# wejoncy/QLLM

Hardware: AMD Instinct MI355X
Metric: decode_tokens_per_s_llama2_7b_w4a16_g128_linear_stack (higher is better)
Workload: dtype f16; 1 GPU; llama2-7b-awq-w4-g128-decode-b1; pack_mode=GEMM, bits=4, group_size=128, layers=32, linears_per_layer=7, batch=1, driven_through=q_layer modules (sibling groups installed by the loader), grouped_qkv_gateup=True, weight_layout=native strip-major copy built on device at first use (qllm_repack_native), graph=True, parallelism=replicas x1, ranks_seen=1, device=gfx950, compute_units=256

## Files before the change

qllm_amd/csrc/capi.hip:

```cpp
#include <stdarg.h>
#include <stdio.h>
#include <string.h>

#include <algorithm>

#include "planner.hpp"

namespace qllm {

static thread_local char g_err[512] = {0};

int set_error(int code, const char *fmt, ...) {
  va_list ap;
  va_start(ap, fmt);
  vsnprintf(g_err, sizeof(g_err), fmt, ap);
  va_end(ap);
  return code;
}
void clear_error() { g_err[0] = 0; }
const char *last_error_text() { return g_err; }

static int native_shape_ok(int bits, int K, int N, int group_size, bool packed_zeros) {
  if (bits != 4 && bits != 3) return set_error(QLLM_ERR_UNSUPPORTED, "the native layout holds 3- and 4-bit weights (got %d)", bits);
  if (K % 32 != 0 || N % 16 != 0) return set_error(QLLM_ERR_UNSUPPORTED, "the native layout needs K %% 32 == 0 and N %% 16 == 0 (K=%d N=%d)", K, N);
// ... 21 lines not shown
    if (w->g_idx) return set_error(QLLM_ERR_INVALID, "the native layout has no act-order (g_idx must be NULL: sort the rows by group first)");
    if (w->layout == QLLM_LAYOUT_NATIVE_F16Z && !w->qzeros) return set_error(QLLM_ERR_INVALID, "NATIVE_F16Z layout needs fp16 qzeros");
  } else {
    if ((w->K * w->bits) % 32 != 0) return set_error(QLLM_ERR_INVALID, "in_features*bits must be a multiple of 32 (K=%d bits=%d)", w->K, w->bits);
    if (w->layout == QLLM_LAYOUT_HQQ && !w->qzeros) return set_error(QLLM_ERR_INVALID, "HQQ layout needs fp16 qzeros");
    if (w->layout == QLLM_LAYOUT_HQQ && w->g_idx) return set_error(QLLM_ERR_INVALID, "HQQ layout has no act-order (g_idx must be NULL)");
    if (w->layout == QLLM_LAYOUT_GPTQ && w->qzeros && (w->N * w->bits) % 32 != 0)
      return set_error(QLLM_ERR_INVALID, "out_features*bits must be a multiple of 32 for packed zeros (N=%d bits=%d)", w->N, w->bits);
  }
  if (w->add_zero_bias < 0 || w->add_zero_bias > 1) return set_error(QLLM_ERR_INVALID, "add_zero_bias must be 0 or 1");
  return QLLM_OK;
}

static int check_io(const void *x, const void *y, int M, int act_dtype) {
  if (!x || !y) return set_error(QLLM_ERR_INVALID, "x / y must not be NULL");
  if (M <= 0) return set_error(QLLM_ERR_INVALID, "M must be >= 1 (got %d)", M);
  if (act_dtype != QLLM_F16 && act_dtype != QLLM_BF16) return set_error(QLLM_ERR_INVALID, "act_dtype must be f16 or bf16");
  if ((uintptr_t)x % 16 != 0) return set_error(QLLM_ERR_INVALID, "x must be 16-byte aligned");
  return QLLM_OK;
}

static int check_quant_layer(const char *required, bool missing, int32_t w_dtype, int32_t N, int32_t K, int32_t group_size) {
  if (missing) return set_error(QLLM_ERR_INVALID, "%s must not be NULL", required);
  if (w_dtype != QLLM_F16 && w_dtype != QLLM_BF16 && w_dtype != QLLM_F32) return set_error(QLLM_ERR_INVALID, "w_dtype must be QLLM_F16, QLLM_BF16 or QLLM_F32");
  if (N <= 0 || K <= 0 || group_size <= 0) return set_error(QLLM_ERR_INVALID, "bad N/K/group_size (%d/%d/%d)", N, K, group_size);
  return QLLM_OK;
}
static int check_whole_groups(int32_t K, int32_t group_size) {
  if (K % group_size != 0) return set_error(QLLM_ERR_INVALID, "K must be a multiple of group_size (K=%d group_size=%d)", K, group_size);
  return QLLM_OK;
}
static int elem_size(int32_t w_dtype) { return w_dtype == QLLM_F32 ? 4 : 2; }
static const char *const kElemAligned = "every buffer must be aligned to its element size";

static int check_workspace(const char *entry, const void *workspace, size_t workspace_bytes, size_t need) {
  if ((need && !workspace) || workspace_bytes < need || (uintptr_t)workspace % 16)
    return set_error(QLLM_ERR_WORKSPACE, "%s needs a 16-byte aligned workspace of %zu bytes (got %zu)", entry, need, workspace ? workspace_bytes : (size_t)0);
  return QLLM_OK;
}

static uint64_t *g_timeline = nullptr;
static int g_timeline_slots = 0, g_timeline_next = 0;

static size_t usable_ws(const void *workspace, size_t workspace_bytes) {
  return (workspace && (uintptr_t)workspace % 256 == 0) ? workspace_bytes : 0;
}
static void carve(void *workspace, int **counters, float **slabs) {
  *counters = (int *)workspace;
  *slabs = (float *)((char *)workspace + kCounterBytes);
}
static void set_split(GemmParams &p, int S, void *workspace, int tail_from = 0, int tail_split = 0) {
  p.split_k = S;
  p.tail_from = tail_split > 1 ? tail_from : 0;
  p.tail_split = tail_split > 1 ? tail_split : 0;
  p.counters = nullptr;
  p.slabs = nullptr;
  if (S > 1 || tail_split > 1) carve(workspace, &p.counters, &p.slabs);
}
static void fill_launch_params(GemmParams &p, const qllm_weight_t *w, const void *x, void *y, int M, int act_dtype) {
  fill_gemm_params(p, w, x, y, M, act_dtype);
#ifdef QLLM_LAB
  p.dbg = g_timeline;
#endif
}

static int fill_strip1_params(Strip1Params &p, const qllm_weight_t *w, void *const *y, int n, const void *x, int M, int act_dtype) {
  fill_call(p, w[0], x, M, act_dtype);
  p.T = w[0].K / 32;
  p.n_groups = w[0].K / w[0].group_size;
  p.group64 = w[0].group_size == 64;
  p.bits3 = w[0].bits == 3;
  int max_strips = 0;
  for (int i = 0; i < n; ++i) {
    fill_layer(p.prob[i], w[i], y[i]);
    p.prob[i].n_strips = w[i].N / 16;
    max_strips = std::max(max_strips, p.prob[i].n_strips);
  }
  return max_strips;
}
static int run_strip1(const StripPlan &pl, const qllm_weight_t *w, void *const *y, int n, const void *x, int M, int act_dtype, hipStream_t stream) {
  Strip1Params p;
  const int max_strips = fill_strip1_params(p, w, y, n, x, M, act_dtype);
  p.dbg = (g_timeline && g_timeline_next < g_timeline_slots) ? g_timeline + 24 * (g_timeline_next++) : nullptr;
  return launch_strip1(p, pl.one_nw, pl.one_maxs, n, max_strips, stream);
}

static int run_strip(const StripPlan &pl, const qllm_weight_t *w, void *const *y, int n, const void *x, int M, int act_dtype, hipStream_t stream) {
  if (pl.one_nw) return run_strip1(pl, w, y, n, x, M, act_dtype, stream);
  StripParams p;
  fill_call(p, w[0], x, M, act_dtype);
  p.n_prob = n;
  p.K = w[0].K;
  p.T = w[0].K / 32;
  p.cpl = pl.cpl;
  p.bits = w[0].bits;
  p.nw = pl.nw;
  p.spw = pl.spw;
  p.ra = pl.ra;
  p.sm = pl.sm;
  p.n_groups = (w[0].K + w[0].group_size - 1) / w[0].group_size;
  p.group_size = w[0].group_size;
  p.dbg = (pl.sm && (!pl.ra || pl.ra == 2) && p.bits == 4 && p.group_size == 128 && g_timeline && g_timeline_next < g_timeline_slots)
              ? g_timeline + 24 * (g_timeline_next++) : nullptr;
  int block = 0;
  for (int i = 0; i < n; ++i) {
    StripProblem &q = p.prob[i];
    fill_layer(q, w[i], y[i]);
    q.N = w[i].N;
    q.n_strips = (w[i].N / 16 + pl.cpl - 1) / pl.cpl;
    q.block_begin = block;
    p.block_begin8[i] = block;
    block += q.n_strips;
  }
  return launch_strip(p, block, stream);
}

static int run_skinny(const qllm_weight_t *w, void *const *y, int n, const void *x, int M, int act_dtype, void *workspace,
                      size_t workspace_bytes, hipStream_t stream) {
  const SkinnyPlan s = plan_skinny(w, n, M);
  if (s.tiles_total > (int)(kCounterBytes / sizeof(int))) return set_error(QLLM_ERR_UNSUPPORTED, "too many column tiles (%d)", s.tiles_total);

  SkinnyParams p;
  fill_call(p, w[0], x, M, act_dtype);
  p.n_prob = n;
  p.K = w[0].K;
  p.T = w[0].K / 32;
  p.group_size = w[0].group_size;
  size_t slab_off = kCounterBytes;
  int tile_off = 0, block = 0;
  for (int i = 0; i < n; ++i) {
    SkinnyProblem &q = p.prob[i];
    fill_layer(q, w[i], y[i]);
    q.N = w[i].N;
    q.n_tiles = (w[i].N + s.tile_cols - 1) / s.tile_cols;
    q.S = s.S;
    q.spw = s.spw;
    q.block_begin = block;
    q.counters = (int *)workspace + tile_off;
    q.slabs = (float *)((char *)workspace + slab_off);
    tile_off += q.n_tiles;
    block += q.n_tiles * s.S;
    if (s.S > 1) slab_off += align_up((size_t)s.S * M * w[i].N * sizeof(float), 256);
  }
  if (s.S > 1) {
    if (!workspace) return set_error(QLLM_ERR_WORKSPACE, "split-K needs a workspace (call qllm_workspace_bytes)");
    if (workspace_bytes < slab_off) return set_error(QLLM_ERR_WORKSPACE, "workspace too small: need %zu bytes, have %zu", slab_off, workspace_bytes);
    if ((uintptr_t)workspace % 256 != 0) return set_error(QLLM_ERR_INVALID, "workspace must be 256-byte aligned");
  }
  return launch_skinny(p, w[0].layout, s.awq_w, block, stream);
}

static const char kNotPrefillKernel[] = "QLLM_F16_IN_BF16_OUT: M=%d K=%d N=%d is not served by the 256x128 prefill kernel";
static int run_tile_gemm(GemmParams &p, int layout, void *workspace, size_t workspace_bytes, hipStream_t stream, bool bf16_out_only = false) {
  const TileChoice c = choose_tile(p, layout, usable_ws(workspace, workspace_bytes));
  if (bf16_out_only && c.kernel != 3) return set_error(QLLM_ERR_UNSUPPORTED, kNotPrefillKernel, p.M, p.K, p.N);
  set_split(p, c.split_k, workspace, c.tail_from, c.tail_split);
  if (c.kernel == 2 && p.N % 128 != 0)
    return set_error(QLLM_ERR_WORKSPACE, "N %% 128 == 64 with bf16 activations converted to fp16: the workspace must hold the copy (call qllm_workspace_bytes_act)");
  if (c.kernel == 2) return launch_gemm2(p, layout, stream);
  if (bf16_out_only) p.out_bf16 = 1;
  if (c.native_bf16) {
    p.native_bf16 = 1;
    p.act_bf16 = 0;
  } else if (p.act_bf16) {
    void *xh = (char *)workspace + c.copy_off;
    if (int rc = launch_bf16_to_f16(p.x, xh, (size_t)p.M * p.K, stream)) return rc;
// ... 459 lines not shown
```

qllm_amd/csrc/kernels.hpp:

```cpp
#pragma once
#include "common.hpp"

namespace qllm {

int launch_dequant(const qllm_weight_t &w, int zero_kind, void *out, int out_dtype, int out_transposed, hipStream_t stream);
int launch_unpack_qweight(const void *qweight, int layout, int bits, int K, int N, int32_t *q_kn, hipStream_t stream);
int launch_pack_qweight(const int32_t *q_kn, int layout, int bits, int K, int N, void *qweight, hipStream_t stream);

int launch_ort_dequant(const void *qweight, const void *scales, const void *qzeros, int zeros_f16, const int32_t *g_idx,
                       int block, int K, int N, void *out, hipStream_t stream);

constexpr int kMaxProblems = 8;

struct SkinnyProblem {
  const uint32_t *qweight;
  const half_t *scales;
  const void *qzeros;
  const half_t *bias;
  void *y;
  float *slabs;
  int *counters;
  int N;
  int n_tiles;
  int S;
// ... 46 lines not shown
  int n_groups;
  int sm;
  uint64_t *dbg;
};
bool strip_group_ok(int group_size, bool strip_major, int bits);
int strip_nw(int K, int strips_total, int compute_units);
int strip_sm_nw(int K, int M, int group_size, int bits);
int strip_spw(int K, int group_size, int nw);
int strip_maxs(int nw, int spw, int cpl, int ra, int sm);
int strip_xl(int nw, int M, int spw, int cpl, int sm);
size_t strip_lds_bytes(int M, int spw, int nw, int cpl, int group_size, int ra, int sm);
int strip_cpl(int cols_total, bool all_mult64, bool all_mult32, int compute_units);
bool strip_x_ok(int M, int spw, int nw, int cpl, int sm);
int launch_strip(const StripParams &p, int grid, hipStream_t stream);
int launch_strip_sm(const StripParams &p, int grid, hipStream_t stream);
int launch_strip_sm_ra(const StripParams &p, int grid, hipStream_t stream);
int launch_strip_dma_g32(const StripParams &p, int grid, hipStream_t stream);
int launch_strip_dma_g64(const StripParams &p, int grid, hipStream_t stream);
int launch_strip_dma_g128(const StripParams &p, int grid, hipStream_t stream);

struct Strip1Problem {
  const uint32_t *qweight;
  const half_t *scales;
  const void *qzeros;
  const half_t *bias;
  void *y;
  int n_strips;
  int zero_kind;
};
struct Strip1Params {
  const void *x;
  int T;
  int n_groups;
  int group64;
  int M;
  int bits3;
  int add_zero_bias;
  int act_bf16;
  uint64_t *dbg;
  Strip1Problem prob[kMaxProblems];
  void *const *ar_peers;
  int *ar_status;
  int ar_rank, ar_world;
  uint32_t ar_slot_bytes;
};

constexpr int kBitGemvMaxM = 16;
struct BitGemvParams {
  const void *x;
  const uint32_t *qweight;
  const half_t *scales;
  const void *qzeros;
  const half_t *bias;
  void *y;
  float *slabs;
  int *counters;
  int M, K, N, group_size, zero_kind, add_zero_bias, act_bf16;
  int ksplit;
  int n_col_blocks, chunk_units;
};
bool bitgemv_ok(const qllm_weight_t &w, int M);
int bitgemv_split(int M, int K, int N);
int bitgemv_cols();
int launch_bitgemv(const BitGemvParams &p, int bits, hipStream_t stream);

constexpr int kCommMaxWorld = 16;
struct CommCtl {
  uint32_t flag[2][kCommMaxWorld];
  uint32_t epoch;
  uint32_t ticket;
};
__device__ __forceinline__ void store16_sys(void *p, uint4_t v) {
  __hip_atomic_store((uint64_t *)p, ((uint64_t)v.y << 32) | v.x, __ATOMIC_RELAXED, __HIP_MEMORY_SCOPE_SYSTEM);
  __hip_atomic_store((uint64_t *)p + 1, ((uint64_t)v.w << 32) | v.z, __ATOMIC_RELAXED, __HIP_MEMORY_SCOPE_SYSTEM);
}
__device__ __forceinline__ uint4_t load16_sys(const void *p) {
  const uint64_t a = __hip_atomic_load((const uint64_t *)p, __ATOMIC_RELAXED, __HIP_MEMORY_SCOPE_SYSTEM);
  const uint64_t b = __hip_atomic_load((const uint64_t *)p + 1, __ATOMIC_RELAXED, __HIP_MEMORY_SCOPE_SYSTEM);
  return uint4_t{(uint32_t)a, (uint32_t)(a >> 32), (uint32_t)b, (uint32_t)(b >> 32)};
}
bool strip1_shape(int K, int blocks, int cus, int *nw, int *maxs, bool odd64 = false);
int launch_strip1(const Strip1Params &p, int nw, int maxs, int n_prob, int max_strips, hipStream_t stream);
int launch_strip1_allreduce(const Strip1Params &p, int nw, int maxs, int n_strips, hipStream_t stream);

int launch_repack_native(const qllm_weight_t &src, int zero_kind, void *qweight_out, void *scales_out, void *qzeros_out, hipStream_t stream);
int launch_unpack_native(const qllm_weight_t &src, int dst_layout, void *qweight_out, void *scales_out, void *qzeros_out, hipStream_t stream);

bool gather_columns_ok(int K);
int launch_gather_columns(const void *x, const int32_t *perm, void *out, int M, int K, hipStream_t stream);

struct GemmParams {
  const void *x;
  const uint32_t *qweight;
  const half_t *scales;
  const void *qzeros;
  const int32_t *g_idx;
  const half_t *bias;
  void *y;
  int M, K, N, group_size, gs_shift, add_zero_bias, zero_kind, act_bf16, n_groups;
  int raster;
  int stagger;
  int out_bf16;
  int sm;
  int split_k;
  float *slabs;
  int *counters;
  int tail_from, tail_split;
  int n_prob, total_tiles;
  struct GemmProb {
    const uint32_t *qweight;
    const half_t *scales;
    const void *qzeros;
    const half_t *bias;
    void *y;
    int N, zero_kind, tile_begin, pad_;
  } prob[4];
  int native_bf16;
  int prio;
  uint64_t *dbg;
};
int launch_gemm(const GemmParams &p, int layout, hipStream_t stream);

bool gemm2_ok(const GemmParams &p, int layout);
int gemm2_split_k(int M, int N, int K);
constexpr int kGemm3MaxProb = 4;
using GemmProb = GemmParams::GemmProb;
int gemm3_tail_split(int M, int N, int K, int *tail_from);
int gemm3_tail_split_tiles(int tiles, int K, int *tail_from, bool uneven = false);
bool gemm3_bf16_native(int layout);
int gemm2_tile_n(int M, int N, int split_k);
size_t gemm2_slab_bytes(int M, int N, int S);
int launch_gemm2(const GemmParams &p, int layout, hipStream_t stream);

struct PanelProblem {
  const uint32_t *qweight;
  const half_t *scales;
  const void *qzeros;
  const half_t *bias;
  void *y;
  int N, zero_kind, panel_begin, pad_;
};
struct PanelParams {
  const void *x;
  int M, K, n_groups, group_size, bits, add_zero_bias, act_bf16, n_prob, split_k, abl, n_panels;
  float *slabs;
  int *counters;
  PanelProblem prob[kMaxProblems];
};
bool panel_shape_ok(int M, int K, int N, int group_size, int bits);
int panel_mt(int M);
int panel_kh(int M);
int panel_split_k(int M, int n_panels, int K);
size_t panel_slab_bytes(int M, int n_panels, int S);
int launch_panel(const PanelParams &p, hipStream_t stream);

constexpr int kGemm3Rows3Bit = 100;
bool gemm3_ok(const GemmParams &p, int layout);
bool gemm3_n_tail(const GemmParams &p, int layout);
inline int gemm3_tile_cols(int N) { return (N + 127) / 128 * 128; }
int gemm3_split_k(int M, int N, int K);
int launch_gemm3(const GemmParams &p, int layout, hipStream_t stream);
int launch_bf16_to_f16(const void *src, void *dst, size_t n, hipStream_t stream);

bool hqq_quant_shape_ok(int N, int K, int bits, int group_size);
size_t hqq_quant_workspace_bytes(int N, int K, int group_size, int iters);
int launch_hqq_quantize(const void *w_nk, int w_dtype, int N, int K, int bits, int group_size, int iters, float lp_norm, float beta, float kappa,
// ... 23 lines not shown
```

qllm_amd/csrc/planner.hip:

```cpp
#include <stdio.h>
#include <stdlib.h>
#include <string.h>

#include <algorithm>

#include "planner.hpp"

namespace qllm {

static int env_int(const char *name, int dflt) {
  const char *v = getenv(name);
  return (v && *v) ? atoi(v) : dflt;
}
static Settable kSettable[] = {
    {"QLLM_STRIP1_3BIT", 0, 1, 0, 0},
    {"QLLM_STRIP1_MAX_M", 1, 4, 0, 0},
    {"QLLM_STRIP1", 0, 2, 0, 0},
    {"QLLM_PANEL", 0, 1, 0, 0},
    {"QLLM_PANEL_MIN_M", 17, 129, 0, 0},
    {"QLLM_PANEL_GROUP_MIN_M", 17, 129, 0, 0},
    {"QLLM_GEMM2", 0, 1, 0, 0},
    {"QLLM_GEMM3", 0, 1, 0, 0},
    {"QLLM_GEMM2_MIN_M", 33, 1 << 30, 0, 0},
    {"QLLM_GEMM3_MIN_M", 0, 1 << 30, 0, 0},
    {"QLLM_GEMM2_SPLITK", 0, 1, 0, 0},
    {"QLLM_GEMM3_TAIL", 0, 1, 0, 0},
    {"QLLM_GEMM3_GROUP", 0, 1, 0, 0},
    {"QLLM_GEMM3_BF16", 0, 1, 0, 0},
    {"QLLM_SKINNY_MAX_M", 0, 64, 0, 0},
    {"QLLM_STRIP_MIN", 0, 1 << 20, 0, 0},
    {"QLLM_BITGEMV", 0, 1, 0, 0},
};
int g_knob_overrides = 0;
Settable *find_knob(const char *name) {
  for (Settable &k : kSettable)
    if (strcmp(k.name, name) == 0) return &k;
  return nullptr;
}
void reset_knobs() {
  for (Settable &k : kSettable) k.set = 0;
  __atomic_store_n(&g_knob_overrides, 0, __ATOMIC_RELAXED);
}
int knob_override(const char *name, int dflt) {
  for (const Settable &k : kSettable)
    if (k.set && strcmp(k.name, name) == 0) return k.value;
  return dflt;
}
#ifdef QLLM_LAB
int knob(const char *name, int dflt) { return g_knob_overrides ? knob_override(name, env_int(name, dflt)) : env_int(name, dflt); }
#endif
int compute_units() {
  static int v = [] {
    int e = env_int("QLLM_NUM_CU", 0);
    if (e > 0) return e;
    int dev = 0, n = 0;
    if (hipGetDevice(&dev) == hipSuccess && hipDeviceGetAttribute(&n, hipDeviceAttributeMultiprocessorCount, dev) == hipSuccess && n > 0) return n;
    (void)hipGetLastError();
    return kNumCU;
  }();
  return v;
}
static int skinny_target_waves() { return knob("QLLM_SKINNY_WAVES", 2048); }
static int skinny_awq_w(int M) { return (M <= 16 && knob("QLLM_SKINNY_AWQ_W", 1) == 2) ? 2 : 1; }
static int skinny_max_m() { return std::min(knob("QLLM_SKINNY_MAX_M", 64), 64); }
static int strip_min_strips() {
  return knob("QLLM_STRIP_MIN", 8);
}

static bool ptrs_aligned(const qllm_weight_t &w) {
  return (uintptr_t)w.qweight % 16 == 0 && (uintptr_t)w.scales % 16 == 0 && (!w.qzeros || (uintptr_t)w.qzeros % 8 == 0);
}
static bool fused_common_ok(const qllm_weight_t &w) {
  return !is_native(w) && w.bits == 4 && w.N % 8 == 0 && w.group_size % 8 == 0 && ptrs_aligned(w);
}
static bool skinny_ok(const qllm_weight_t &w, int M) {
  return M <= skinny_max_m() && fused_common_ok(w) && w.K % 32 == 0 && w.g_idx == nullptr;
}
static bool gemm_ok(const qllm_weight_t &w) {
  if (!fused_common_ok(w) || w.K % 64 != 0) return false;
  if (w.layout == QLLM_LAYOUT_AWQ_GEMM) return w.group_size % 4 == 0;
  if (w.g_idx) {
    const int groups = (w.K + w.group_size - 1) / w.group_size;
    return (size_t)groups * 128 * 4 + 65536 <= 160 * 1024;
  }
  return true;
}
static int layout_family(const qllm_weight_t &w) { return is_native(w) ? 2 : (w.layout == QLLM_LAYOUT_AWQ_GEMM ? 1 : 0); }

void fill_gemm_params(GemmParams &p, const qllm_weight_t *w, const void *x, void *y, int M, int act_dtype) {
  fill_call(p, *w, x, M, act_dtype);
  fill_layer(p, *w, y);
  p.g_idx = w->g_idx;
  p.K = w->K;
  p.N = w->N;
  p.group_size = w->group_size;
  p.gs_shift = ((w->group_size & (w->group_size - 1)) == 0) ? __builtin_ctz((unsigned)w->group_size) : -1;
  p.n_groups = (w->K + w->group_size - 1) / w->group_size;
  p.sm = is_native(*w) ? 1 : 0;
  p.split_k = 1;
// ... 116 lines not shown
  for (int ci = 0; ci < n_cands; ++ci) {
    const int c = cands[ci];
    if (!dma_fits(c)) continue;
    int blocks = 0;
    for (int i = 0; i < n; ++i) blocks += (w[i].N / 16 + c - 1) / c;
    const double cost = (double)((blocks + cus - 1) / cus) * (96.0 * 1024 + x_bytes + c * strip_bytes);
    if (best == 0 || cost < best_cost * 0.97) { best = c; best_cost = cost; }
    if (c == dma_cpl) { best = c; break; }
  }
  const int cpl = best ? best : 1;
  const bool g32_ra = g32 && cpl == 1 && M <= 8 && K <= 4096;
  const int nw = (cpl == 1 && M <= 16) ? 16 : 8;
  const int spw = (strip_spw(K, gs, nw) + 1) & ~1;
  if (g32_ra || strip_lds_bytes(M, spw, nw, cpl, gs, 2, 1) > 156 * 1024) return false;
  return take(plan, cpl, nw, spw, 2, 1);
}

static void upgrade_to_strip1(const qllm_weight_t &w, int M, int strips, StripPlan *plan) {
  int nw1 = 0, maxs1 = 0;
  const int s1 = knob("QLLM_STRIP1", 1);
  const bool w4 = w.bits == 4 && (w.group_size == 128 || (w.group_size == 64 && s1 != 2 && w.K <= 24576));
  const bool w3 = w.bits == 3 && (w.group_size == 128 || w.group_size == 64) && w.K <= 16384 && knob("QLLM_STRIP1_3BIT", 1);
  if (M == 1 && (w4 || w3) && s1 && strip1_shape(w.K, strips, compute_units(), &nw1, &maxs1, w4 && w.group_size == 64)) {
    plan->one_nw = nw1;
    plan->one_maxs = maxs1;
  }
}
static bool plan_strip_native(const qllm_weight_t *w, int M, const StripCols &c, bool after_dma, StripPlan *plan) {
  const int K = w[0].K, gs = w[0].group_size, bits = w[0].bits;
  const bool g32 = gs == 32;
  const bool longk = strip_longk(w[0]);
  const int slab_nw = strip_ra_base(M) ? 0 : strip_sm_nw(K, M, gs, bits);
  const int sm_ra_cpl4 = knob("QLLM_SM_RA_CPL4", 1);
  const int cpl = (!after_dma && sm_ra_cpl4 && !g32 && slab_nw == 0 && M >= 5 && M <= 16 && c.m64 && c.cols / 64 >= compute_units() / 2) ? (bits == 3 ? 2 : 4) : 1;
  int nw = after_dma ? (M > 16 ? 8 : 16) : ((M > 16 || cpl > 1) ? 8 : (slab_nw ? slab_nw : 16));
  for (int tries = 0; tries < 2; ++tries) {
    const int spw = strip_spw(K, gs, nw);
    const int ra = (slab_nw == 0 || (longk && nw == 16)) ? 1 : 0;
    if (!ra && K / 32 < strip_maxs(nw, spw, 1, 0, 1)) return false;
    if ((ra || strip_x_ok(M, spw, nw, 1, 1)) && strip_lds_bytes(M, spw, nw, cpl, gs, ra, 1) <= 156 * 1024) {
      upgrade_to_strip1(w[0], M, c.cols / 16, plan);
      return take(plan, cpl, nw, spw, ra, 1);
    }
    if (nw == 16 || M > 16 || cpl > 1) break;
    nw = 16;
  }
  return false;
}

static bool plan_strip_rowstream(const qllm_weight_t *w, int M, const StripCols &c, StripPlan *plan) {
  const int K = w[0].K, gs = w[0].group_size, bits = w[0].bits, cus = compute_units();
  const int ra_base = strip_ra_base(M);
  const bool longk = strip_longk(w[0]);
  int force_cpl = knob("QLLM_STRIP_CPL", 0);
  int first = (bits == 3 || M > 16) ? 1 : strip_cpl(c.cols, c.m64, c.m32 && M <= 4, cus);
  if (M > 16) force_cpl = 1;
  if (force_cpl == 4 && c.m64 && bits == 4) first = 4;
  if (force_cpl == 2 && c.m32 && bits == 4) first = 2;
  if (force_cpl == 1) first = 1;
  const int cand_cpl[2] = {first, 1};
  for (int ci = 0; ci < 2; ++ci) {
    const int cpl = cand_cpl[ci];
    if (ci >= 1 && cpl == cand_cpl[ci - 1]) continue;
    const int strips = c.cols / (16 * cpl);
    if (cpl == 1 && strips < strip_min_strips()) continue;
    int nw = cpl == 4 ? 8 : ((cpl == 2 || bits == 3) ? 16 : strip_nw(K, strips, cus));
    if (M > 16) nw = 8;
    for (int tries = 0; tries < 2; ++tries) {
      const int spw = strip_spw(K, gs, nw);
      const int ra = (ra_base || (longk && cpl == 1 && nw == 16)) ? 1 : 0;
      if ((ra || strip_x_ok(M, spw, nw, cpl, 0)) && strip_lds_bytes(M, spw, nw, cpl, gs, ra, 0) <= 156 * 1024) return take(plan, cpl, nw, spw, ra, 0);
      if (nw == 16 || M > 16 || cpl == 4) break;
      nw = 16;
    }
  }
  return false;
}

bool strip_plan(const qllm_weight_t *w, int n, int M, StripPlan *plan) {
  *plan = StripPlan{};
  StripCols c;
  if (M > strip_row_limit(w, n) || panel_takes_instead(w, n, M) || !strip_layers_ok(w, n, M, &c)) return false;
  if (!is_native(w[0])) return plan_strip_rowstream(w, M, c, plan);
  if (plan_strip1_rows4(w, M, c.cols / 16, plan)) return true;
  const bool dma = strip_dma_applies(w, n, M);
  if (dma && plan_strip_dma(w, n, M, plan)) return true;
  return plan_strip_native(w, M, c, dma, plan);
}

SkinnyPlan plan_skinny(const qllm_weight_t *w, int n, int M) {
  SkinnyPlan s;
  s.awq_w = skinny_awq_w(M);
  s.tile_cols = skinny_tile_cols(w[0].layout, s.awq_w);
  s.tiles_total = 0;
  for (int i = 0; i < n; ++i) s.tiles_total += (w[i].N + s.tile_cols - 1) / s.tile_cols;
  skinny_plan(w[0].K, M, s.tiles_total, skinny_target_waves(), &s.S, &s.spw);
  return s;
}

static bool split_fits(size_t ws_bytes, size_t slab_bytes, int counters) {
  return ws_bytes >= kCounterBytes + slab_bytes && counters <= (int)(kCounterBytes / sizeof(int));
}
int gemm3_split_for(int M, int N, int K, size_t ws_bytes) {
  const int S = gemm3_split_k(M, N, K);
  if (S <= 1 || !split_fits(ws_bytes, gemm2_slab_bytes(M, gemm3_tile_cols(N), S), tiles_256x128(M, gemm3_tile_cols(N)))) return 1;
  return S;
}
static int gemm2_split_for(int M, int N, int K, size_t ws_bytes) {
  const int S = gemm2_split_k(M, N, K);
  if (S <= 1 || !split_fits(ws_bytes, gemm2_slab_bytes(M, N, S), tiles_256x128(M, N))) return 1;
  return S;
}
int panel_split_for(int M, int n_panels, int K, size_t ws_bytes) {
  const int S = panel_split_k(M, n_panels, K);
  if (S <= 1 || !split_fits(ws_bytes, panel_slab_bytes(M, n_panels, S), n_panels)) return 1;
  return S;
}
int bitgemv_split_for(int M, int K, int N, size_t ws_bytes) {
  const int S = bitgemv_split(M, K, N);
  if (S <= 1 || !split_fits(ws_bytes, (size_t)S * M * N * sizeof(float), (N + 15) / 16)) return 1;
  return S;
}
static size_t gemm3_tail_slab_bytes(int tail_tiles, int TS) { return TS > 1 ? (size_t)tail_tiles * TS * 256 * 128 * sizeof(float) : 0; }
static int tail_that_fits(int TS, int tiles, size_t ws_bytes, int *tail_from) {
  if (TS > 1 && split_fits(ws_bytes, gemm3_tail_slab_bytes(tiles - *tail_from, TS), tiles - *tail_from)) return TS;
  *tail_from = tiles;
  return 1;
}
static int gemm3_tail_for(int M, int N, int K, size_t ws_bytes, int *tail_from) {
  return tail_that_fits(gemm3_tail_split(M, N, K, tail_from), tiles_256x128(M, gemm3_tile_cols(N)), ws_bytes, tail_from);
}
static int group_tiles(const qllm_weight_t *w, int n, int M) {
  int t = 0;
  for (int i = 0; i < n; ++i) t += tiles_256x128(M, w[i].N);
  return t;
}
int tile_group_tail_for(const qllm_weight_t *w, int n, int M, size_t ws_bytes, int *tail_from) {
  const int tiles = group_tiles(w, n, M);
  return tail_that_fits(gemm3_tail_split_tiles(tiles, w[0].K, tail_from), tiles, ws_bytes, tail_from);
}

static size_t bf16_copy_bytes(int M, int K, int act_bf16) { return act_bf16 ? align_up((size_t)M * K * 2, 256) : 0; }

TileChoice choose_tile(const GemmParams &p, int layout, size_t ws_bytes) {
  GemmParams q = p;
  q.act_bf16 = 0;
  if (gemm3_ok(q, layout)) {
    const int S3 = gemm3_split_for(p.M, p.N, p.K, ws_bytes);
    if (gemm2_split_k(p.M, p.N, p.K) == 1 || S3 > 1) {
      const int native = p.act_bf16 && gemm3_bf16_native(layout);
      const size_t copy = native ? 0 : bf16_copy_bytes(p.M, p.K, p.act_bf16);
      const int tiles = tiles_256x128(p.M, gemm3_tile_cols(p.N));
      int tail_from = tiles;
      const int TS = S3 > 1 ? 1 : gemm3_tail_for(p.M, p.N, p.K, ws_bytes > copy ? ws_bytes - copy : 0, &tail_from);
      const size_t used = kCounterBytes + (S3 > 1 ? align_up(gemm2_slab_bytes(p.M, gemm3_tile_cols(p.N), S3), 256) : align_up(gemm3_tail_slab_bytes(tiles - tail_from, TS), 256));
      if (!copy || ws_bytes >= used + copy) return TileChoice{3, S3, used, tail_from, TS, native};
    }
  }
  return TileChoice{2, gemm2_split_for(p.M, p.N, p.K, ws_bytes), 0, 0, 0, 0};
}

static bool native_prefill_ok(const qllm_weight_t *w, GemmParams &p) {
  if (!ptrs_aligned(*w)) return false;
  if (panel_serves(w, p.M)) return true;
  if (w->bits == 3) return gemm3_ok(p, kGemm3Rows3Bit);
  if (w->bits != 4) return false;
  if (gemm2_ok(p, QLLM_LAYOUT_GPTQ)) return true;
  GemmParams q = p;
  q.act_bf16 = 0;
  return gemm3_n_tail(q, QLLM_LAYOUT_GPTQ) && gemm3_ok(q, QLLM_LAYOUT_GPTQ);
}

static Decision routed(Route r, int layout = 0) {
  Decision d;
  memset(&d, 0, sizeof(d));
  d.route = r;
  d.layout = layout;
  return d;
}
static Decision refused(int rc) {
  Decision d = routed(ROUTE_NONE);
  d.rc = rc;
  return d;
}

Decision decide_single(const qllm_weight_t *w, int M, int act_dtype) {
  Decision d = routed(ROUTE_STRIP);
  GemmParams p;
  fill_gemm_params(p, w, nullptr, nullptr, M, act_dtype);
  if ((w->bits == 3 || is_native(*w)) && strip_plan(w, 1, M, &d.strip)) return d;
  if (is_native(*w)) {
    if (!native_prefill_ok(w, p))
      return refused(set_error(QLLM_ERR_UNSUPPORTED, "native-layout layer: no fused kernel for M=%d K=%d N=%d g=%d bits=%d (decode sizes, and M > 64 with "
                               "K %% 64 == 0, N %% 128 == 0 and a power-of-two group size, are served)", M, w->K, w->N, w->group_size, w->bits));
    if (panel_serves(w, M)) return routed(ROUTE_PANEL);
    if (w->bits == 3) return routed(ROUTE_ROWS3, kGemm3Rows3Bit);
    return routed(ROUTE_TILE, QLLM_LAYOUT_GPTQ);
  }
  if (skinny_ok(*w, M)) {
    if (strip_plan(w, 1, M, &d.strip)) return d;
    if (M > 32 && gemm_ok(*w) && gemm2_ok(p, w->layout)) return routed(ROUTE_TILE, w->layout);
    return routed(ROUTE_SKINNY);
  }
  if (w->bits == 3 && M > 64 && w->layout != QLLM_LAYOUT_AWQ_GEMM && !w->g_idx && ptrs_aligned(*w) && gemm3_ok(p, kGemm3Rows3Bit))
    return routed(ROUTE_ROWS3, kGemm3Rows3Bit);
  if (gemm_ok(*w)) return routed(gemm2_ok(p, w->layout) ? ROUTE_TILE : ROUTE_GEMM, w->layout);
  if (knob("QLLM_BITGEMV", 1) && bitgemv_ok(*w, M)) return routed(ROUTE_BITGEMV);
  return refused(set_error(QLLM_ERR_UNSUPPORTED, "no fused kernel for bits=%d K=%d N=%d g=%d layout=%d act_order=%d; use qllm_dequant + GEMM",
                           w->bits, w->K, w->N, w->group_size, w->layout, w->g_idx != nullptr));
}

static bool tile_group_serves(const qllm_weight_t *w, int n, int M, int act_dtype) {
  if (!knob("QLLM_GEMM3_GROUP", 1) || !knob("QLLM_GEMM3", 1) || n < 2 || n > kGemm3MaxProb || M < 384) return false;
  const int gs = w[0].group_size;
  if (w[0].bits != 4 || w[0].K % 64 != 0 || gs < 32 || (gs & (gs - 1)) != 0) return false;
  if (act_dtype == QLLM_BF16 && !gemm3_bf16_native(QLLM_LAYOUT_GPTQ)) return false;
  for (int i = 0; i < n; ++i) {
    if (w[i].layout == QLLM_LAYOUT_AWQ_GEMM || w[i].g_idx || w[i].N % 128 != 0 || is_native(w[i]) != is_native(w[0])) return false;
    if (!ptrs_aligned(w[i])) return false;
    if ((size_t)M * w[i].K * 2 >= 0x7fffffffull || (size_t)w[i].K * w[i].N / 2 >= 0x7fffffffull) return false;
  }
  return group_tiles(w, n, M) >= compute_units();
}

Decision decide_group(const qllm_weight_t *w, int n, int M, int act_dtype) {
  for (int i = 0; i < n; ++i) {
    if (w[i].K != w[0].K || w[i].group_size != w[0].group_size || w[i].bits != w[0].bits || layout_family(w[0]) != layout_family(w[i]) ||
        w[i].add_zero_bias != w[0].add_zero_bias)
      return refused(set_error(QLLM_ERR_INVALID, "grouped weights must agree on K, group_size, bits, layout family and add_zero_bias"));
  }
  if (tile_group_serves(w, n, M, act_dtype)) return routed(ROUTE_TILE_GROUP, QLLM_LAYOUT_GPTQ);
  for (int i = 0; i < n; ++i) {
    if (w[i].bits == 3 || is_native(w[i])) continue;
    if (!skinny_ok(w[i], M))
      return refused(set_error(QLLM_ERR_UNSUPPORTED, "grouped forward needs the decode kernel (4-bit, M<=%d, K%%32==0, no act-order)", skinny_max_m()));
  }
  Decision d = routed(ROUTE_STRIP);
  if (strip_plan(w, n, M, &d.strip)) return d;
  if (panel_group_serves(w, n, M)) return routed(ROUTE_PANEL);
  if (is_native(w[0]))
    return refused(set_error(QLLM_ERR_UNSUPPORTED, "grouped forward: native-layout layers are served for M <= 32 (4 bits: <= 128) with group size 64 / 128 (4 bits: also 32), and 4-bit groups of at least one 256x128 tile per CU from 384 rows (M=%d g=%d)", M, w[0].group_size));
  if (w[0].bits != 4) return refused(set_error(QLLM_ERR_UNSUPPORTED, "grouped forward: no fused kernel for %d-bit weights in this shape", w[0].bits));
  return routed(ROUTE_SKINNY);
}

void describe(const Decision &d, const qllm_weight_t *w, int n, int M, size_t ws_bytes, char *buf, size_t buflen) {
  const char *sm = is_native(w[0]) ? " layout=strip-major" : "";
  switch (d.route) {
    case ROUTE_STRIP: {
      const StripPlan &pl = d.strip;
      if (pl.one_nw)
        snprintf(buf, buflen, "strip1 nw=%d round=%d%s%s%s grid=strips x %d layout=strip-major", pl.one_nw, pl.one_maxs,
                 pl.one_nw * pl.one_maxs == w[0].K / 32 ? " exact" : "", w[0].group_size == 64 ? (w[0].bits == 3 ? " g64 bits=3" : " g64") : (w[0].bits == 3 ? " bits=3" : ""),
                 M > 1 ? " rows=4" : "", n);
      else
        snprintf(buf, buflen, "strip nw=%d cpl=%d spw=%d form=%s row_tiles=%d%s", pl.nw, pl.cpl, pl.spw,
                 pl.ra == 2 ? "dma-A" : (pl.ra ? "register-A" : "lds-slab"), M > 32 ? 4 : (M > 16 ? 2 : 1), pl.sm ? " layout=strip-major" : "");
      return;
    }
    case ROUTE_PANEL: {
      char layers[24] = "";
      if (n > 1) snprintf(layers, sizeof(layers), " layers=%d", n);
      snprintf(buf, buflen, "panel cols=64 row_tiles=%d k_halves=%d split_k=%d%s%s layout=strip-major", panel_mt(M), panel_kh(M),
               panel_split_for(M, panels_of(w, n), w[0].K, ws_bytes), layers, w[0].bits == 3 ? " bits=3" : "");
      return;
    }
    case ROUTE_ROWS3: {
      const int S = gemm3_split_for(M, w[0].N, w[0].K, ws_bytes);
      if (S > 1) snprintf(buf, buflen, "gemm3 tile=256x128 matrix-waves=8 staging-waves=4 bits=3 split_k=%d%s", S, sm);
      else snprintf(buf, buflen, "gemm3 tile=256x128 matrix-waves=8 staging-waves=4 bits=3%s", sm);
      return;
    }
    case ROUTE_TILE: {
      GemmParams p;
      fill_gemm_params(p, &w[0], nullptr, nullptr, M, QLLM_F16);
      const TileChoice c = choose_tile(p, d.layout, ws_bytes);
      const char *nt = w[0].N % 128 ? " n_tail=64" : "";
      if (c.kernel == 3 && c.tail_split > 1) snprintf(buf, buflen, "gemm3 tile=256x128 matrix-waves=8 staging-waves=4 tail_split=%d%s%s", c.tail_split, nt, sm);
      else if (c.kernel == 3 && c.split_k > 1) snprintf(buf, buflen, "gemm3 tile=256x128 matrix-waves=8 staging-waves=4 split_k=%d%s%s", c.split_k, nt, sm);
      else if (c.kernel == 3) snprintf(buf, buflen, "gemm3 tile=256x128 matrix-waves=8 staging-waves=4%s%s", nt, sm);
      else snprintf(buf, buflen, "gemm2 tile=256x%d split_k=%d%s", gemm2_tile_n(M, w[0].N, c.split_k), c.split_k, sm);
      return;
    }
    case ROUTE_TILE_GROUP: {
      int tail_from = 0;
      const int TS = tile_group_tail_for(w, n, M, ws_bytes, &tail_from);
      if (TS > 1) snprintf(buf, buflen, "gemm3 tile=256x128 matrix-waves=8 staging-waves=4 layers=%d tail_split=%d%s", n, TS, sm);
      else snprintf(buf, buflen, "gemm3 tile=256x128 matrix-waves=8 staging-waves=4 layers=%d%s", n, sm);
      return;
    }
    case ROUTE_GEMM: snprintf(buf, buflen, "gemm tile=128x128%s", w[0].g_idx ? " act-order-gather" : ""); return;
    case ROUTE_SKINNY: {
      const SkinnyPlan s = plan_skinny(w, n, M);
      snprintf(buf, buflen, "skinny tile_cols=%d split_k=%d spw=%d", s.tile_cols, s.S, s.spw);
      return;
    }
    case ROUTE_BITGEMV:
      snprintf(buf, buflen, "bitgemv bits=%d cols=%d waves=8 split_k=%d", w[0].bits, bitgemv_cols(), bitgemv_split_for(M, w[0].K, w[0].N, ws_bytes));
      return;
    default: snprintf(buf, buflen, "unsupported (%s)", last_error_text()[0] ? last_error_text() : "dequant + GEMM");
  }
}

size_t workspace_bytes_act(const qllm_weight_t *w, int M, int act_dtype) {
  if (!w || M <= 0) return kCounterBytes;
  size_t tiles = 0;
  if (M > 32) {
    GemmParams p;
    fill_gemm_params(p, w, nullptr, nullptr, M, QLLM_F16);
    p.g_idx = nullptr;
    const bool g3 = gemm3_ok(p, w->bits == 3 ? kGemm3Rows3Bit : (w->layout == QLLM_LAYOUT_AWQ_GEMM ? QLLM_LAYOUT_AWQ_GEMM : QLLM_LAYOUT_GPTQ));
    int tail_from = 0;
    const int TS = g3 && w->bits != 3 ? gemm3_tail_split(M, w->N, w->K, &tail_from) : 1;
    const size_t tail = align_up(gemm3_tail_slab_bytes(tiles_256x128(M, gemm3_tile_cols(w->N)) - tail_from, TS), 256);
    const size_t split3 = g3 ? align_up(gemm2_slab_bytes(M, gemm3_tile_cols(w->N), gemm3_split_k(M, w->N, w->K)), 256) : 0;
    tiles = std::max(std::max(align_up(gemm2_slab_bytes(M, w->N, gemm2_split_k(M, w->N, w->K)), 256), split3), tail) +
            (g3 ? bf16_copy_bytes(M, w->K, act_dtype == QLLM_BF16) : 0);
    if (M > 128) return kCounterBytes + tiles;
  }
  if (M >= 9 && M <= 128 && w->N % 64 == 0) tiles = std::max(tiles, align_up(panel_slab_bytes(M, w->N / 64, panel_split_k(M, w->N / 64, w->K)), 256));
  if (M > 64) return kCounterBytes + tiles;
  const size_t slabs = align_up((size_t)skinny_max_split(M) * M * w->N * sizeof(float), 256);
  return kCounterBytes + (tiles > slabs ? tiles : slabs);
}

}
```

qllm_amd/csrc/planner.hpp:

```cpp
#pragma once
#include <string.h>

#include "kernels.hpp"

namespace qllm {

constexpr size_t kCounterBytes = 16384;
inline size_t align_up(size_t v, size_t a) { return (v + a - 1) / a * a; }
const char *last_error_text();

struct Settable {
  const char *name;
  int lo, hi;
  int value, set;
};
Settable *find_knob(const char *name);
void reset_knobs();
inline int panel_ablation() { return knob("QLLM_PANEL_ABL", 0); }

inline bool is_native(const qllm_weight_t &w) { return w.layout == QLLM_LAYOUT_NATIVE || w.layout == QLLM_LAYOUT_NATIVE_F16Z; }
inline int zero_kind_of(const qllm_weight_t &w) {
  if (w.layout == QLLM_LAYOUT_HQQ || w.layout == QLLM_LAYOUT_NATIVE_F16Z) return ZK_F16;
  if (w.qzeros == nullptr) return ZK_SYM;
  return ZK_PACKED;
}
template <typename Params>
inline void fill_call(Params &p, const qllm_weight_t &w0, const void *x, int M, int act_dtype) {
  memset(&p, 0, sizeof(p));
  p.x = x;
  p.M = M;
  p.add_zero_bias = w0.add_zero_bias;
  p.act_bf16 = (act_dtype == QLLM_BF16);
}
template <typename Problem>
inline void fill_layer(Problem &q, const qllm_weight_t &w, void *y) {
  q.qweight = (const uint32_t *)w.qweight;
  q.scales = (const half_t *)w.scales;
  q.qzeros = w.qzeros;
  q.bias = (const half_t *)w.bias;
  q.y = y;
  q.zero_kind = zero_kind_of(w);
}
inline int tiles_256x128(int M, int cols) { return ((M + 255) / 256) * (cols / 128); }
void fill_gemm_params(GemmParams &p, const qllm_weight_t *w, const void *x, void *y, int M, int act_dtype);

struct StripPlan {
  int cpl, nw, spw, ra, sm;
  int one_nw, one_maxs;
};
bool strip_plan(const qllm_weight_t *w, int n, int M, StripPlan *plan);

struct SkinnyPlan {
  int awq_w, tile_cols, tiles_total, S, spw;
};
SkinnyPlan plan_skinny(const qllm_weight_t *w, int n, int M);

struct TileChoice {
  int kernel;
  int split_k;
  size_t copy_off;
  int tail_from, tail_split;
  int native_bf16;
};
TileChoice choose_tile(const GemmParams &p, int layout, size_t ws_bytes);

int gemm3_split_for(int M, int N, int K, size_t ws_bytes);
int panel_split_for(int M, int n_panels, int K, size_t ws_bytes);
int bitgemv_split_for(int M, int K, int N, size_t ws_bytes);
int tile_group_tail_for(const qllm_weight_t *w, int n, int M, size_t ws_bytes, int *tail_from);

enum Route { ROUTE_NONE = 0, ROUTE_STRIP, ROUTE_PANEL, ROUTE_ROWS3, ROUTE_TILE, ROUTE_GEMM, ROUTE_SKINNY, ROUTE_BITGEMV, ROUTE_TILE_GROUP };
struct Decision {
  Route route;
  StripPlan strip;
  int layout;
  int rc;
};
Decision decide_single(const qllm_weight_t *w, int M, int act_dtype);
Decision decide_group(const qllm_weight_t *w, int n, int M, int act_dtype);
void describe(const Decision &d, const qllm_weight_t *w, int n, int M, size_t ws_bytes, char *buf, size_t buflen);
size_t workspace_bytes_act(const qllm_weight_t *w, int M, int act_dtype);

}
```

Baseline: 1155 tokens/s.

## Add strip1 walk kernel issuing all grouped members' weight loads at once

Adds a specialised strip1 kernel for grouped launches of two or three 4-bit g128 members (QKV, gate/up). Each block loads every member's weights, scales and zeros into registers up front, then reuses one prepared activation slab in LDS across all members. The goal is more memory-level parallelism and less repeated activation preparation in decode GEMV. The cost is higher register and LDS pressure, plus extra template instantiations. The planner enables it by default through a knob.

```diff
diff --git a/qllm_amd/csrc/capi.hip b/qllm_amd/csrc/capi.hip
--- a/qllm_amd/csrc/capi.hip
+++ b/qllm_amd/csrc/capi.hip
@@ -127,6 +127,7 @@
   Strip1Params p;
   const int max_strips = fill_strip1_params(p, w, y, n, x, M, act_dtype);
   p.dbg = (g_timeline && g_timeline_next < g_timeline_slots) ? g_timeline + 24 * (g_timeline_next++) : nullptr;
+  if (pl.one_walk > 0 && !p.dbg) return launch_strip1_walk(p, pl.one_nw, pl.one_maxs, n, max_strips, stream);
   return launch_strip1(p, pl.one_nw, pl.one_maxs, n, max_strips, stream);
 }
 
diff --git a/qllm_amd/csrc/kernels.hpp b/qllm_amd/csrc/kernels.hpp
--- a/qllm_amd/csrc/kernels.hpp
+++ b/qllm_amd/csrc/kernels.hpp
@@ -152,6 +152,8 @@
 bool strip1_shape(int K, int blocks, int cus, int *nw, int *maxs, bool odd64 = false);
 int launch_strip1(const Strip1Params &p, int nw, int maxs, int n_prob, int max_strips, hipStream_t stream);
 int launch_strip1_allreduce(const Strip1Params &p, int nw, int maxs, int n_strips, hipStream_t stream);
+bool strip1_walk_serves(int nw, int maxs, int n_prob, int bits, int group_size);
+int launch_strip1_walk(const Strip1Params &p, int nw, int maxs, int n_prob, int max_strips, hipStream_t stream);
 
 int launch_repack_native(const qllm_weight_t &src, int zero_kind, void *qweight_out, void *scales_out, void *qzeros_out, hipStream_t stream);
 int launch_unpack_native(const qllm_weight_t &src, int dst_layout, void *qweight_out, void *scales_out, void *qzeros_out, hipStream_t stream);
diff --git a/qllm_amd/csrc/planner.hip b/qllm_amd/csrc/planner.hip
--- a/qllm_amd/csrc/planner.hip
+++ b/qllm_amd/csrc/planner.hip
@@ -15,6 +15,7 @@
 static Settable kSettable[] = {
     {"QLLM_STRIP1_3BIT", 0, 1, 0, 0},
     {"QLLM_STRIP1_MAX_M", 1, 4, 0, 0},
+    {"QLLM_STRIP1_WALK", 0, 1, 0, 0},
     {"QLLM_STRIP1", 0, 2, 0, 0},
     {"QLLM_PANEL", 0, 1, 0, 0},
     {"QLLM_PANEL_MIN_M", 17, 129, 0, 0},
@@ -297,10 +298,13 @@
   StripCols c;
   if (M > strip_row_limit(w, n) || panel_takes_instead(w, n, M) || !strip_layers_ok(w, n, M, &c)) return false;
   if (!is_native(w[0])) return plan_strip_rowstream(w, M, c, plan);
-  if (plan_strip1_rows4(w, M, c.cols / 16, plan)) return true;
-  const bool dma = strip_dma_applies(w, n, M);
-  if (dma && plan_strip_dma(w, n, M, plan)) return true;
-  return plan_strip_native(w, M, c, dma, plan);
+  bool ok = plan_strip1_rows4(w, M, c.cols / 16, plan);
+  if (!ok) {
+    const bool dma = strip_dma_applies(w, n, M);
+    ok = (dma && plan_strip_dma(w, n, M, plan)) || plan_strip_native(w, M, c, dma, plan);
+  }
+  if (ok && plan->one_nw && strip1_walk_serves(plan->one_nw, plan->one_maxs, n, w[0].bits, w[0].group_size)) plan->one_walk = knob("QLLM_STRIP1_WALK", 1) ? 1 : -1;
+  return ok;
 }
 
 SkinnyPlan plan_skinny(const qllm_weight_t *w, int n, int M) {
@@ -465,9 +469,9 @@
     case ROUTE_STRIP: {
       const StripPlan &pl = d.strip;
       if (pl.one_nw)
-        snprintf(buf, buflen, "strip1 nw=%d round=%d%s%s%s grid=strips x %d layout=strip-major", pl.one_nw, pl.one_maxs,
+        snprintf(buf, buflen, "strip1 nw=%d round=%d%s%s%s grid=strips x %d%s layout=strip-major", pl.one_nw, pl.one_maxs,
                  pl.one_nw * pl.one_maxs == w[0].K / 32 ? " exact" : "", w[0].group_size == 64 ? (w[0].bits == 3 ? " g64 bits=3" : " g64") : (w[0].bits == 3 ? " bits=3" : ""),
-                 M > 1 ? " rows=4" : "", n);
+                 M > 1 ? " rows=4" : "", n, pl.one_walk < 0 ? " per-member" : "");
       else
         snprintf(buf, buflen, "strip nw=%d cpl=%d spw=%d form=%s row_tiles=%d%s", pl.nw, pl.cpl, pl.spw,
                  pl.ra == 2 ? "dma-A" : (pl.ra ? "register-A" : "lds-slab"), M > 32 ? 4 : (M > 16 ? 2 : 1), pl.sm ? " layout=strip-major" : "");
diff --git a/qllm_amd/csrc/planner.hpp b/qllm_amd/csrc/planner.hpp
--- a/qllm_amd/csrc/planner.hpp
+++ b/qllm_amd/csrc/planner.hpp
@@ -47,6 +47,7 @@
 struct StripPlan {
   int cpl, nw, spw, ra, sm;
   int one_nw, one_maxs;
+  int one_walk;
 };
 bool strip_plan(const qllm_weight_t *w, int n, int M, StripPlan *plan);
 
diff --git a/qllm_amd/csrc/strip1_walk.hip b/qllm_amd/csrc/strip1_walk.hip
--- /dev/null
+++ b/qllm_amd/csrc/strip1_walk.hip
@@ -0,0 +1,40 @@
+#include "strip1_walk_kernel.hpp"
+
+namespace qllm {
+
+bool strip1_walk_serves(int nw, int maxs, int n_prob, int bits, int group_size) {
+  if (n_prob < 2 || n_prob > 3 || bits != 4 || group_size != 128) return false;
+  return (nw == 4 && maxs == 8) || (nw == 4 && maxs == 16) || (nw == 7 && maxs == 16) || (nw == 8 && maxs == 16);
+}
+
+template <int NW, int MAXS, bool EXACT, int NP, int MR>
+static int launch_t(const Strip1Params &p, int max_strips, hipStream_t stream) {
+  constexpr int lds_bytes = strip1_walk_lds_bytes<NW, MAXS, NP, MR>();
+  static_assert(lds_bytes <= 64 * 1024, "no opt-in needed");
+  hipLaunchKernelGGL((strip1_walk_kernel<NW, MAXS, EXACT, NP, MR>), dim3(max_strips), dim3(NW * 64), lds_bytes, stream, p);
+  QLLM_HIP_CHECK(hipGetLastError());
+  return QLLM_OK;
+}
+
+template <int NW, int MAXS>
+static int launch_e(const Strip1Params &p, int n_prob, int max_strips, hipStream_t stream) {
+  const bool exact = NW * MAXS == p.T;
+  if (p.M > 1) {
+    if (n_prob == 2) return exact ? launch_t<NW, MAXS, true, 2, 4>(p, max_strips, stream) : launch_t<NW, MAXS, false, 2, 4>(p, max_strips, stream);
+    return exact ? launch_t<NW, MAXS, true, 3, 4>(p, max_strips, stream) : launch_t<NW, MAXS, false, 3, 4>(p, max_strips, stream);
+  }
+  if (n_prob == 2) return exact ? launch_t<NW, MAXS, true, 2, 1>(p, max_strips, stream) : launch_t<NW, MAXS, false, 2, 1>(p, max_strips, stream);
+  return exact ? launch_t<NW, MAXS, true, 3, 1>(p, max_strips, stream) : launch_t<NW, MAXS, false, 3, 1>(p, max_strips, stream);
+}
+
+int launch_strip1_walk(const Strip1Params &p, int nw, int maxs, int n_prob, int max_strips, hipStream_t stream) {
+  if (strip1_walk_serves(nw, maxs, n_prob, p.bits3 ? 3 : 4, p.group64 ? 64 : 128) && p.M >= 1 && p.M <= 4) {
+    if (nw == 4 && maxs == 8) return launch_e<4, 8>(p, n_prob, max_strips, stream);
+    if (nw == 4 && maxs == 16) return launch_e<4, 16>(p, n_prob, max_strips, stream);
+    if (nw == 7 && maxs == 16) return launch_e<7, 16>(p, n_prob, max_strips, stream);
+    if (nw == 8 && maxs == 16) return launch_e<8, 16>(p, n_prob, max_strips, stream);
+  }
+  return set_error(QLLM_ERR_UNSUPPORTED, "internal: no walk instantiation for nw=%d round=%d layers=%d", nw, maxs, n_prob);
+}
+
+}
diff --git a/qllm_amd/csrc/strip1_walk_kernel.hpp b/qllm_amd/csrc/strip1_walk_kernel.hpp
--- /dev/null
+++ b/qllm_amd/csrc/strip1_walk_kernel.hpp
@@ -0,0 +1,191 @@
+#pragma once
+#include "strip1_kernel.hpp"
+
+namespace qllm {
+
+template <int NW, int MAXS, int NP, int MR = 1>
+constexpr int strip1_walk_lds_bytes() {
+  constexpr int XL = (MAXS * 4 + 63) / 64;
+  return NP * 16 * MR * strip1_rs(NW) * 4 + NW * (MR * XL * 1024 + 256);
+}
+
+template <int NW, int MAXS, bool EXACT, int NP, int MR, bool ALL>
+__device__ __forceinline__ void strip1_walk_block(const Strip1Params &p, const Strip1Problem (&pr)[NP], const bool (&live)[NP], const int add_zero_bias, const int act_bf16, float *lds) {
+  constexpr int NCH = 2;
+  constexpr int NG = MAXS / 4;
+  constexpr int XL = (MAXS * 4 + 63) / 64;
+  constexpr int RS = strip1_rs(NW);
+  constexpr int RED = 16 * MR * RS;
+  const int lane = threadIdx.x & 63;
+  const int wave = __builtin_amdgcn_readfirstlane(threadIdx.x >> 6);
+  const int g = lane >> 4, i = lane & 15;
+  const int b = blockIdx.x;
+
+  const int T = p.T;
+  const int t0 = wave * MAXS;
+  const int tb = EXACT ? t0 : min(t0, T - MAXS);
+  uint4_t xa[MR][XL];
+  bool xkeep[XL];
+#pragma unroll
+  for (int u = 0; u < XL; ++u) {
+    const int c = lane + 64 * u;
+    const int cc = min(c, MAXS * 4 - 1);
+#pragma unroll
+    for (int m = 0; m < MR; ++m) {
+      xa[m][u] = uint4_t{0, 0, 0, 0};
+      if (MR == 1 || m < p.M) xa[m][u] = *(const uint4_t *)((const uint16_t *)p.x + (size_t)m * 32 * T + 32 * tb + 8 * cc);
+    }
+    const int t = tb + (c >> 2);
+    xkeep[u] = EXACT ? (c < MAXS * 4) : (c < MAXS * 4 && t >= t0 && t < T);
+  }
+  const int G0 = tb / 4;
+  const size_t grow = (size_t)b * p.n_groups + G0;
+  const int gj = min(g, NG - 1);
+  half_t sc[NP];
+  uint32_t zraw[NP], w[NP][MAXS];
+#pragma unroll
+  for (int m = 0; m < NP; ++m) {
+    if (ALL || live[m]) {
+      const int zk = pr[m].zero_kind;
+      const uint32_t *zbase = (zk == ZK_SYM) ? (const uint32_t *)pr[m].scales : (const uint32_t *)pr[m].qzeros;
+      const int zmul = (zk == ZK_PACKED) ? 2 : 8;
+      const int zoff = (zk == ZK_PACKED) ? (i >> 3) : (i >> 1);
+      sc[m] = pr[m].scales[(grow + gj) * 16 + i];
+      zraw[m] = zbase[(grow + gj) * zmul + zoff];
+      const uint32_t *wl = pr[m].qweight + ((size_t)b * T + tb) * 64 + lane;
+#pragma unroll
+      for (int s = 0; s < MAXS; ++s) w[m][s] = __builtin_nontemporal_load(wl + s * 64);
+    }
+  }
+  __builtin_amdgcn_sched_barrier(0);
+
+  char *wbase = (char *)lds + NP * RED * 4 + wave * (MR * XL * 1024 + 256);
+  char *zeros = wbase + MR * XL * 1024;
+
+  float sx[MR][XL], sxp[MR][XL];
+#pragma unroll
+  for (int m = 0; m < MR; ++m)
+#pragma unroll
+    for (int u = 0; u < XL; ++u) asm volatile("" : "+v"(xa[m][u]));
+  *(uint32_t *)(zeros + 4 * lane) = 0u;
+#pragma unroll
+  for (int m = 0; m < MR; ++m)
+#pragma unroll
+    for (int u = 0; u < XL; ++u) {
+      const half8_t zero8 = {0, 0, 0, 0, 0, 0, 0, 0};
+      half8_t xv = act_bf16 ? bf16x8_to_h8(xa[m][u]) : __builtin_bit_cast(half8_t, xa[m][u]);
+      xv = xkeep[u] ? xv : zero8;
+      const half8_t pv = a_perm_04152637(xv);
+      const half2_t p0 = {pv[0], pv[1]}, p1 = {pv[2], pv[3]}, p2 = {pv[4], pv[5]}, p3 = {pv[6], pv[7]};
+      const half2_t d16 = half2_t{(half_t)0.0625f, (half_t)0.0625f};
+      const half2_t q0 = p0, q1 = p1 * d16, q2 = p2, q3 = p3 * d16;
+      const half2_t one = {(half_t)1.f, (half_t)1.f};
+      float a = __builtin_amdgcn_fdot2(p0, one, 0.f, false);
+      a = __builtin_amdgcn_fdot2(p1, one, a, false);
+      a = __builtin_amdgcn_fdot2(p2, one, a, false);
+      a = __builtin_amdgcn_fdot2(p3, one, a, false);
+      float c = __builtin_amdgcn_fdot2(q0, one, 0.f, false);
+      c = __builtin_amdgcn_fdot2(q1, one, c, false);
+      c = __builtin_amdgcn_fdot2(q2, one, c, false);
+      c = __builtin_amdgcn_fdot2(q3, one, c, false);
+      a = dpp_add1<0xB1>(a); c = dpp_add1<0xB1>(c);
+      a = dpp_add1<0x4E>(a); c = dpp_add1<0x4E>(c);
+      a = dpp_add1<0x141>(a); c = dpp_add1<0x141>(c);
+      a = dpp_add1<0x140>(a); c = dpp_add1<0x140>(c);
+      sx[m][u] = a; sxp[m][u] = c;
+      *(half8_t *)(wbase + m * (XL * 1024) + 16 * (lane + 64 * u)) = half8_t{q0.x, q0.y, q1.x, q1.y, q2.x, q2.y, q3.x, q3.y};
+    }
+
+  uint32_t a_addr[NG];
+  const uint32_t xs_lane = (uint32_t)(wbase - (char *)lds) + 16 * g, z_lane = (uint32_t)(zeros - (char *)lds) + 16 * g;
+#pragma unroll
+  for (int j = 0; j < NG; ++j)
+    a_addr[j] = ((i >> 2) == (j & 3)) ? xs_lane + (MR > 1 ? (i & 3) * (XL * 1024) : 0) : z_lane - 64 * 4 * j;
+  const uint32_t mask_lo = nib_mask_vgpr();
+  const uint32_t mask_hi = mask_lo << 4;
+
+#pragma unroll
+  for (int m = 0; m < NP; ++m) {
+    if (!ALL && !live[m]) continue;
+    const int zk = pr[m].zero_kind;
+    const uint32_t zsel_p = (zk == ZK_PACKED) ? 0xffffffffu : 0u, zsel_h = (zk == ZK_F16) ? 0xffffffffu : 0u;
+    const uint32_t zsel_s = (zk == ZK_SYM) ? __builtin_bit_cast(uint32_t, 8.0f) : 0u;
+    const uint32_t zr = zraw[m];
+    const float zp = (float)(((zr >> (4 * (i & 7))) + (uint32_t)add_zero_bias) & 15u);
+    const float zh = (float)__builtin_bit_cast(half_t, (uint16_t)((i & 1) ? (zr >> 16) : (zr & 0xffffu)));
+    const float zf = __builtin_bit_cast(float, (__builtin_bit_cast(uint32_t, zp) & zsel_p) | (__builtin_bit_cast(uint32_t, zh) & zsel_h) | zsel_s);
+    const float sf = (float)sc[m];
+    float cf[MR];
+#pragma unroll
+    for (int r = 0; r < MR; ++r) cf[r] = sf * __builtin_fmaf(zf, sx[r][0], 1024.f * sxp[r][0]);
+
+    float4_t acc[NCH];
+#pragma unroll
+    for (int s = 0; s < MAXS; ++s) {
+      const int j = s / 4, ch = s % NCH;
+      const half8_t av = *(const half8_t *)((const char *)lds + a_addr[j] + 64 * s);
+      const uint32_t wv = w[m][s], w8 = wv >> 8;
+      const half2_t b0 = as_h2((wv & mask_lo) | kMagic), b1 = as_h2((wv & mask_hi) | kMagic);
+      const half2_t b2 = as_h2((w8 & mask_lo) | kMagic), b3 = as_h2((w8 & mask_hi) | kMagic);
+      const half8_t bf = {b0.x, b0.y, b1.x, b1.y, b2.x, b2.y, b3.x, b3.y};
+      const float4_t cin = (s < NCH) ? float4_t{0.f, 0.f, 0.f, 0.f} : acc[ch];
+      acc[ch] = __builtin_amdgcn_mfma_f32_16x16x32_f16(av, bf, cin, 0, 0, 0);
+    }
+
+    float *red = lds + m * RED;
+#pragma unroll
+    for (int r = 0; r < MR; ++r) {
+      float a = acc[0][MR > 1 ? r : 0];
+#pragma unroll
+      for (int ch = 1; ch < NCH; ++ch) a += acc[ch][MR > 1 ? r : 0];
+      const float val = 0.f + __builtin_fmaf(sf, a, -cf[r]);
+      red[(r * 16 + i) * RS + wave * 4 + g] = val;
+    }
+    __syncthreads();
+    if (threadIdx.x < 16 * MR) {
+      const float4_t *row = (const float4_t *)(red + threadIdx.x * RS);
+      float4_t t[NW];
+#pragma unroll
+      for (int q = 0; q < NW; ++q) t[q] = row[q];
+#pragma unroll
+      for (int st = 1; st < NW; st *= 2)
+#pragma unroll
+        for (int q = 0; q + st < NW; q += 2 * st) t[q] = t[q] + t[q + st];
+      float v = (t[0][0] + t[0][1]) + (t[0][2] + t[0][3]);
+      const int n = b * 16 + (threadIdx.x & 15), mrow = threadIdx.x >> 4;
+      if (pr[m].bias) v += (float)pr[m].bias[n];
+      if (MR == 1 || mrow < p.M) {
+        const size_t at = (size_t)mrow * pr[m].n_strips * 16 + n;
+        if (act_bf16) ((uint16_t *)pr[m].y)[at] = f32_to_bf16(v);
+        else ((half_t *)pr[m].y)[at] = (half_t)v;
+      }
+    }
+  }
+}
+
+template <int NW, int MAXS, bool EXACT, int NP, int MR = 1>
+__global__ __launch_bounds__(NW * 64, (NP == 2 && MR == 1) ? 6 : 4) void strip1_walk_kernel(const Strip1Params p) {
+  static_assert(MAXS % 4 == 0 && MAXS >= 8 && MAXS <= 16, "one pass of whole 128-wide groups");
+  static_assert(NP == 2 || NP == 3, "two or three members, every load in flight at once");
+  static_assert(MR == 1 || MR == 4, "one batch row, or four");
+  extern __shared__ __attribute__((aligned(16))) float lds[];
+  Strip1Problem pr[NP];
+#pragma unroll
+  for (int m = 0; m < NP; ++m) pr[m] = p.prob[m];
+#pragma unroll
+  for (int m = 0; m < NP; ++m)
+    asm volatile("" ::"s"(pr[m].qweight), "s"(pr[m].scales), "s"(pr[m].qzeros), "s"(pr[m].bias), "s"(pr[m].y), "s"(pr[m].n_strips), "s"(pr[m].zero_kind));
+  asm volatile("" ::"s"(p.x), "s"(p.T), "s"(p.n_groups));
+  int add_zero_bias = p.add_zero_bias, act_bf16 = p.act_bf16;
+  asm volatile("" : "+s"(add_zero_bias), "+s"(act_bf16));
+  bool live[NP], all = true;
+#pragma unroll
+  for (int m = 0; m < NP; ++m) {
+    live[m] = (int)blockIdx.x < pr[m].n_strips;
+    all = all && live[m];
+  }
+  if (all) strip1_walk_block<NW, MAXS, EXACT, NP, MR, true>(p, pr, live, add_zero_bias, act_bf16, lds);
+  else strip1_walk_block<NW, MAXS, EXACT, NP, MR, false>(p, pr, live, add_zero_bias, act_bf16, lds);
+}
+
+}
```

Result: slower. 1124 tokens/s (-2.7%).
